# zkonduit/ezkl

Hardware: AMD Instinct MI355X
Metric: BN254 G1 MSM pts/s (2^20 points per GPU; NTT 2^22 elems/s in extra) (higher is better)
Workload: dtype u32x8 (254-bit modular integer, Montgomery); 1 GPU; configs[1]: standalone 2^20-point BN254 G1 MSM (uniform scalars, try-and-increment bases) + 2^22 scalar-field NTT per GPU; parallelism=points sharded across 1 rank(s); all_gather of 64-B partials + host fold

## Files before the change

### ezkl_amd/csrc/msm.hip

```cpp
#include "common.hpp"
#include <deque>
#include <thread>
#include <chrono>
#include "curve.hpp"
#include "curve29.hpp"
#include "host64.hpp"
#include <string.h>

namespace ezkl {

static constexpr uint32_t MSM_MAX_PART_BITS = 12;
static constexpr uint32_t MSM_SPAN_HEAVY = 16;
static constexpr uint32_t MSM_PART_STAGE = 13312;
static constexpr uint32_t MSM_BINSORT_STAGE = 15360;
static constexpr uint32_t MSM_HEAVY_CHUNK = 256;
static constexpr uint32_t MSM_DIGIT_E = 8;
static constexpr uint32_t MSM_LMIN = 8;
static constexpr uint32_t MSM_MAX_BIG = 64;
static constexpr uint32_t MSM_BIG_BLOCKS = 64;
static constexpr uint32_t MSM_BIG_ROWS = 8;

__device__ __forceinline__ uint32_t msm_part_of(uint32_t bucket, uint32_t NP) { return bucket ? 1u + (bucket & (NP - 1u)) : 0u; }
__device__ __forceinline__ uint32_t msm_lane_len(const uint32_t* offsets, uint32_t nb, uint32_t nlanes, uint32_t lmin) {
    const uint32_t l = (uint32_t)(((uint64_t)offsets[nb] + nlanes - 1) / nlanes);
// ... 155 lines not shown
        uint32_t raw = msm_take_bits(s, c) + carry;
        if (raw > half) {
            carry = 1;
            if (raw != (1u << c)) f(w, (1u << c) - raw - 1u, neg ^ 1u);
        } else {
            carry = 0;
            if (raw) f(w, raw - 1u, neg);
        }
    }
}

__device__ __forceinline__ bool msm_digit_step(fe_t& s, uint32_t neg, uint32_t c, uint32_t& carry, uint32_t& bucket, uint32_t& sign) {
    const uint32_t half = 1u << (c - 1);
    const uint32_t raw = msm_take_bits(s, c) + carry;
    if (raw > half) {
        carry = 1;
        bucket = (1u << c) - raw - 1u;
        sign = neg ^ 1u;
        return raw != (1u << c);
    }
    carry = 0;
    bucket = raw - 1u;
    sign = neg;
    return raw != 0;
}

__device__ __forceinline__ uint32_t msm_block_scan(uint32_t v, uint32_t* wsum, uint32_t& total) {
    const uint32_t lane = threadIdx.x & 63u, wave = threadIdx.x >> 6, nw = blockDim.x >> 6;
    uint32_t x = v;
#pragma unroll
    for (uint32_t d = 1; d < 64; d <<= 1) {
        const uint32_t y = __shfl_up(x, d, 64);
        if (lane >= d) x += y;
    }
    if (lane == 63) wsum[wave] = x;
    __syncthreads();
    if (wave == 0) {
        uint32_t s = lane < nw ? wsum[lane] : 0u;
#pragma unroll
        for (uint32_t d = 1; d < 16; d <<= 1) {
            const uint32_t y = __shfl_up(s, d, 64);
            if (lane >= d) s += y;
        }
        if (lane < nw) wsum[lane] = s;
    }
    __syncthreads();
    total = wsum[nw - 1];
    const uint32_t r = x + (wave ? wsum[wave - 1] : 0u);
    __syncthreads();
    return r;
}

__global__ __launch_bounds__(256) void msm_hist_kernel(const fe_t* scalars, size_t n, size_t per_block, WinPlan wp,
                                                       uint32_t LB, uint32_t NP, uint32_t* wg_hist, uint32_t* wg_cnt,
                                                       const fe_t* const* scal_list, uint32_t* zero_base, uint32_t zero_words, size_t bstride) {
    BOFF(); BSH(wg_hist); BSH(wg_cnt);
    if (scal_list) scalars = scal_list[blockIdx.z];
    if (zero_base) {
        BSH(zero_base);
        for (uint32_t i = blockIdx.x * 256 + threadIdx.x; i < zero_words; i += gridDim.x * 256) zero_base[i] = 0;
    }
    __shared__ uint32_t lh[(1u << MSM_MAX_PART_BITS) + 1];
    const uint32_t NQ = NP + 1;
    for (uint32_t p = threadIdx.x; p < NQ; p += 256) lh[p] = 0;
    __syncthreads();
    size_t lo = (size_t)blockIdx.x * per_block, hi = lo + per_block < n ? lo + per_block : n;
    for (size_t i0 = lo + threadIdx.x; i0 < hi; i0 += 4 * 256) {
        fe_t s[4];
        uint32_t neg[4], carry[4] = {0, 0, 0, 0};
#pragma unroll
        for (int q = 0; q < 4; q++) {
            const size_t i = i0 + (size_t)q * 256;
            if (i < hi) s[q] = msm_canon(scalars, i, neg[q]);
            else { s[q] = Fr::zero(); neg[q] = 0; }
        }
        for (uint32_t w = 0; w < wp.W; w++) {
            const uint32_t c = wp.width(w);
#pragma unroll
            for (int q = 0; q < 4; q++) {
                uint32_t bucket, sign;
                if (msm_digit_step(s[q], neg[q], c, carry[q], bucket, sign)) atomicAdd(&lh[msm_part_of(bucket, NP)], 1u);
            }
        }
    }
    __syncthreads();
    for (uint32_t p = threadIdx.x; p < NQ; p += 256) {
        wg_hist[(size_t)blockIdx.x * NQ + p] = lh[p];
        wg_cnt[(size_t)blockIdx.x * NQ + p] = lh[p];
    }
}
__global__ __launch_bounds__(1024) void msm_hist_scan_kernel(uint32_t* wg_hist, uint32_t G, uint32_t NP, uint32_t* part_count, size_t bstride) {
    BOFF(); BSH(wg_hist); BSH(part_count);
    __shared__ uint32_t sums[32][33];
    const uint32_t c = threadIdx.x & 31, j = threadIdx.x >> 5;
    const uint32_t p = blockIdx.x * 32 + c;
    const uint32_t chunk = (G + 31) / 32, g0 = j * chunk, g1 = g0 + chunk < G ? g0 + chunk : G;
    uint32_t s = 0;
    if (p < NP)
        for (uint32_t g = g0; g < g1; g++) s += wg_hist[(size_t)g * NP + p];
    sums[j][c] = s;
    __syncthreads();
    if (j == 0) {
        uint32_t run = 0;
        for (uint32_t q = 0; q < 32; q++) {
            uint32_t v = sums[q][c];
            sums[q][c] = run;
            run += v;
        }
        if (p < NP) part_count[p] = run;
    }
    __syncthreads();
    if (p < NP) {
        uint32_t run = sums[j][c];
        for (uint32_t g = g0; g < g1; g++) {
            uint32_t v = wg_hist[(size_t)g * NP + p];
            wg_hist[(size_t)g * NP + p] = run;
            run += v;
        }
    }
}
__device__ __forceinline__ void msm_part_scan_body(const uint32_t* part_count, uint32_t NQ, uint32_t* part_base, uint32_t* big_flag,
                                                   uint32_t* big_list, uint32_t* big_count, uint32_t* sh) {
    const uint32_t t = threadIdx.x;
    constexpr uint32_t PER = 5;
    uint32_t v[PER], sum = 0;
#pragma unroll
    for (uint32_t q = 0; q < PER; q++) {
        const uint32_t i = PER * t + q;
        v[q] = i < NQ ? part_count[i] : 0;
        sum += v[q];
    }
    uint32_t total;
    uint32_t run = msm_block_scan(sum, sh, total) - sum;
#pragma unroll
    for (uint32_t q = 0; q < PER; q++) {
        const uint32_t i = PER * t + q;
        if (i < NQ) part_base[i] = run;
        run += v[q];
    }
    if (t == 1023) part_base[NQ] = total;
#pragma unroll
    for (uint32_t q = 0; q < PER; q++) {
        const uint32_t i = PER * t + q;
        if (i == 0 || i >= NQ) continue;
        uint32_t slot = 0;
        if (v[q] > MSM_BINSORT_STAGE) {
            slot = atomicAdd(big_count, 1u);
            if (slot < MSM_MAX_BIG) big_list[slot] = i - 1;
            slot = slot < MSM_MAX_BIG ? slot + 1 : 0;
        }
        big_flag[i - 1] = slot;
    }
}
__global__ __launch_bounds__(1024) void msm_part_scan_kernel(const uint32_t* part_count, uint32_t NQ, uint32_t* part_base, uint32_t* big_flag,
                                                             uint32_t* big_list, uint32_t* big_count, size_t bstride) {
    BOFF(); BSH(part_count); BSH(part_base); BSH(big_flag); BSH(big_list); BSH(big_count);
    __shared__ uint32_t sh[1024];
    msm_part_scan_body(part_count, NQ, part_base, big_flag, big_list, big_count, sh);
}
__global__ __launch_bounds__(1024) void msm_partition_kernel(const fe_t* scalars, size_t n, size_t per_block, WinPlan wp,
                                                             uint32_t LB, uint32_t NP, size_t base_offset, size_t tab_stride,
                                                             const uint32_t* part_base, const uint32_t* wg_hist, const uint32_t* wg_cnt, uint2* entries,
                                                             uint32_t* vals, const fe_t* const* scal_list, size_t bstride) {
    BOFF(); BSH(part_base); BSH(wg_hist); BSH(wg_cnt); BSH(entries); BSH(vals);
    if (scal_list) scalars = scal_list[blockIdx.z];
    extern __shared__ uint32_t plds[];
    __shared__ uint32_t tsum[1024];
    const uint32_t NQ = NP + 1;
    uint32_t* start = plds;
    uint32_t* cursor = plds + (NQ + 1);
    uint32_t* gbase = plds + 2 * (NQ + 1);
    uint2* stage = reinterpret_cast<uint2*>(plds + 3 * (NQ + 1));
    const uint32_t t = threadIdx.x, T = blockDim.x;
    const uint32_t K = (NQ + T - 1) / T;
    uint32_t loc = 0;
    for (uint32_t q = 0; q < K; q++) {
        const uint32_t p = t * K + q;
        if (p < NQ) loc += wg_cnt[(size_t)blockIdx.x * NQ + p];
    }
    uint32_t total;
    uint32_t run = msm_block_scan(loc, tsum, total) - loc;
    for (uint32_t q = 0; q < K; q++) {
        const uint32_t p = t * K + q;
        if (p < NQ) {
            start[p] = run;
            cursor[p] = run;
            gbase[p] = part_base[p] + wg_hist[(size_t)blockIdx.x * NQ + p];
            run += wg_cnt[(size_t)blockIdx.x * NQ + p];
        }
    }
    __syncthreads();
    const size_t lo = (size_t)blockIdx.x * per_block, hi = lo + per_block < n ? lo + per_block : n;
    const size_t i = lo + t;
    if (i < hi) {
        uint32_t neg;
        fe_t s = msm_canon(scalars, i, neg);
        msm_foreach_digit(s, neg, wp, [&](uint32_t w, uint32_t bucket, uint32_t sign) {
            const uint32_t r = atomicAdd(&cursor[msm_part_of(bucket, NP)], 1u);
            stage[r] = make_uint2((uint32_t)(w * tab_stride + base_offset + i) | (sign << 31), bucket);
        });
    }
    __syncthreads();
    const uint32_t PB = 31 - __clz(NP);
    for (uint32_t idx = t; idx < total; idx += T) {
        const uint2 e = stage[idx];
        const uint32_t p = msm_part_of(e.y, NP);
        const uint32_t slot = gbase[p] + (idx - start[p]);
        if (p) entries[slot] = make_uint2(e.x, e.y >> PB);
        else vals[slot] = e.x;
    }
}
__device__ __forceinline__ uint32_t msm_wave_rank(uint32_t* cnt, uint32_t key) {
    const uint64_t active = __ballot(1);
    const uint32_t first = __builtin_amdgcn_readfirstlane(key);
    if (__ballot(key == first) == active) {
        const uint32_t rank = (uint32_t)__popcll(active & ((1ull << (threadIdx.x & 63u)) - 1ull));
        uint32_t base = 0;
        if (rank == 0) base = atomicAdd(&cnt[first], (uint32_t)__popcll(active));
        return (uint32_t)__builtin_amdgcn_readfirstlane(base) + rank;
    }
    return atomicAdd(&cnt[key], 1u);
}
__device__ __forceinline__ void msm_bins_scan(uint32_t* cnt, uint32_t* tsum, uint32_t nbins, uint32_t p, uint32_t beg, const uint32_t* part_base,
                                              bool emit, uint32_t* offsets, g1x29_t* buckets) {
    const uint32_t t = threadIdx.x;
    uint32_t loc[4], s = 0;
#pragma unroll
    for (int q = 0; q < 4; q++) {
        uint32_t j = t * 4 + q;
        loc[q] = j < nbins ? cnt[j] : 0;
        s += loc[q];
    }
    uint32_t total;
    uint32_t run = msm_block_scan(s, tsum, total) - s;
#pragma unroll
    for (int q = 0; q < 4; q++) {
        uint32_t j = t * 4 + q;
        if (j < nbins) {
            cnt[j] = run;
            if (emit) {
                const bool b0 = (p == 0 && j == 0);
                offsets[(size_t)p * nbins + j] = b0 ? part_base[0] : beg + run;
                if (b0 ? part_base[1] == part_base[0] : loc[q] == 0) st_f29(&buckets[(size_t)p * nbins + j].zz, Fq29::zero());
// ... 130 lines not shown
        uint32_t mid = (lo + hi) >> 1;
        if (offsets[mid] <= k0) lo = mid; else hi = mid;
    }
    uint32_t b = lo, bin_end = offsets[b + 1];
    uint32_t end_next = offsets[b + 2 <= nb ? b + 2 : nb];
    lane_first[t] = b;
    bool started_before = offsets[b] < k0;
    g1x29_t acc = g1x29_identity();
    MsmRec nxt = msm_fetch(tab, vals[k0]);
    uint32_t vn = k0 + 1 < k1 ? vals[k0 + 1] : 0u;
    for (uint32_t k = k0; k < k1; k++) {
        if (k == bin_end) {
            if (started_before) st_g1x29(head + t, acc); else st_g1x29(buckets + b, acc);
            acc.zz = Fq29::zero();
            started_before = false;
            b++;
            bin_end = end_next;
            if (bin_end == k) {
                uint32_t probes = 1;
                while (bin_end == k && probes < 4) { b++; bin_end = offsets[b + 1]; probes++; }
                if (bin_end == k) {
                    uint32_t lo2 = b + 1, hi2 = nb;
                    while (hi2 - lo2 > 1) {
                        uint32_t mid = (lo2 + hi2) >> 1;
                        if (offsets[mid] <= k) lo2 = mid; else hi2 = mid;
                    }
                    b = lo2;
                    bin_end = offsets[b + 1];
                }
            }
            end_next = offsets[b + 2 <= nb ? b + 2 : nb];
        }
        const MsmRec cur = nxt;
        nxt = msm_fetch(tab, vn);
        vn = k + 2 < k1 ? vals[k + 2] : 0u;
        acc = g1x29_add_mixed(acc, g1a29_unpack(cur.p), cur.neg);
    }
    if (k1 == bin_end) {
        if (started_before) st_g1x29(head + t, acc); else st_g1x29(buckets + b, acc);
    } else {
        if (started_before) st_g1x29(head + t, acc); else st_g1x29(tail + t, acc);
    }
}
EZ_D g1x29_t g1x29_shfl_down(const g1x29_t& p, uint32_t d) {
    g1x29_t r;
    const uint32_t* s = p.x.v;
    uint32_t* o = r.x.v;
#pragma unroll
    for (int k = 0; k < 36; k++) o[k] = __shfl_down(s[k], d);
    return r;
}
__global__ __launch_bounds__(256) void msm_fixup_boundary_tree_kernel(const uint32_t* offsets, uint32_t nb, uint32_t nlanes,
                                                                      const uint32_t* lane_first, const g1x29_t* head, const g1x29_t* tail, g1x29_t* buckets,
                                                                      uint32_t* heavy_list, uint32_t* heavy_count, uint32_t* chunk_list, uint32_t lmin,
                                                                      uint32_t span_heavy, size_t bstride) {
    BOFF(); BSH(offsets); BSH(lane_first); BSH(head); BSH(tail); BSH(buckets); BSH(heavy_list); BSH(heavy_count); BSH(chunk_list);
    const uint32_t t = blockIdx.x * blockDim.x + threadIdx.x + 1;
    const uint32_t lane = threadIdx.x & 63u;
    const uint32_t L = msm_lane_len(offsets, nb, nlanes, lmin);
    const uint64_t k0 = (uint64_t)t * L;
    bool cut = t < nlanes && k0 < offsets[nb];
    uint32_t b = 0, t1 = 0, t2 = 0;
    if (cut) {
        b = lane_first[t];
        const uint32_t beg = offsets[b], end = offsets[b + 1];
        cut = beg < k0;
        t1 = beg / L; t2 = (end - 1) / L;
    }
    if (cut && t2 - t1 > span_heavy) {
        if (t == t1 + 1 && t2 - t1 > MSM_HEAVY_CHUNK) heavy_list[atomicAdd(heavy_count, 1u)] = b;
        if ((t - t1 - 1) % MSM_HEAVY_CHUNK == 0) chunk_list[atomicAdd(heavy_count + 1, 1u)] = t;
        cut = false;
    }
    const uint32_t wave_last = t + (63u - lane);
    const uint32_t run = cut ? (t2 < wave_last ? t2 : wave_last) - t + 1u : 0u;
    uint32_t longest = run;
#pragma unroll
    for (uint32_t o = 32; o > 0; o >>= 1) {
        const uint32_t m = __shfl_xor(longest, o);
        longest = m > longest ? m : longest;
    }
    if (longest == 0) return;
    if (longest <= 2) {
        if (!cut || t != t1 + 1) return;
        g1x29_t acc = g1x29_add(ld_g1x29(tail + t1), ld_g1x29(head + t));
        for (uint32_t u = t + 1; u <= t2; u++) acc = g1x29_add(acc, ld_g1x29(head + u));
        st_g1x29(buckets + b, acc);
        return;
    }
    g1x29_t v = cut ? ld_g1x29(head + t) : g1x29_identity();
    uint32_t have = cut ? 1u : 0u;
#pragma unroll 1
    for (uint32_t d = 1; d < longest; d <<= 1) {
        const g1x29_t w = g1x29_shfl_down(v, d);
        const uint32_t hw = __shfl_down(have, d);
        if (have == d && run > d) {
            v = g1x29_add(v, w);
            have += hw;
        }
    }
    if (!cut || t != t1 + 1) return;
    g1x29_t acc = g1x29_add(ld_g1x29(tail + t1), v);
    for (uint32_t u = t + run; u <= t2; u++) acc = g1x29_add(acc, ld_g1x29(head + u));
    st_g1x29(buckets + b, acc);
}
__global__ __launch_bounds__(256) void msm_fixup_heavy1_kernel(const uint32_t* offsets, uint32_t nb, uint32_t nlanes, const uint32_t* lane_first, g1x29_t* head,
                                                               const g1x29_t* tail, g1x29_t* buckets, const uint32_t* chunk_list, const uint32_t* counts, uint32_t lmin,
                                                               uint32_t coop, size_t bstride) {
    BOFF(); BSH(offsets); BSH(lane_first); BSH(head); BSH(tail); BSH(buckets); BSH(chunk_list); BSH(counts);
    const uint32_t nchunks = counts[1], L = msm_lane_len(offsets, nb, nlanes, lmin);
    const uint32_t wave = threadIdx.x >> 6, lane = threadIdx.x & 63u;
    for (uint32_t ci = blockIdx.x * 4u + wave; ci < nchunks; ci += gridDim.x * 4u) {
        const uint32_t start = chunk_list[ci], b = lane_first[start];
        const uint32_t t2 = (offsets[b + 1] - 1) / L;
        const uint32_t stop = start + MSM_HEAVY_CHUNK - 1 < t2 ? start + MSM_HEAVY_CHUNK - 1 : t2;
        const uint32_t t1 = offsets[b] / L;
        const bool whole = t2 - t1 <= MSM_HEAVY_CHUNK;
        g1x29_t acc = (whole && lane == 63u) ? ld_g1x29(tail + t1) : g1x29_identity();
        for (uint32_t t = start + lane; t <= stop; t += 64) acc = g1x29_add(acc, ld_g1x29(head + t));
        acc = coop ? g1x29_group_sum_coop(acc, 64) : g1x29_group_sum(acc, 64);
        if (lane == 0) st_g1x29(whole ? buckets + b : head + start, acc);
    }
}
__global__ __launch_bounds__(256) void msm_fixup_heavy2_kernel(const uint32_t* offsets, uint32_t nb, uint32_t nlanes, const g1x29_t* head, const g1x29_t* tail,
                                                               const uint32_t* heavy_list, const uint32_t* counts, g1x29_t* buckets, uint32_t lmin, uint32_t coop, size_t bstride) {
    BOFF(); BSH(offsets); BSH(head); BSH(tail); BSH(heavy_list); BSH(counts); BSH(buckets);
    const uint32_t L = msm_lane_len(offsets, nb, nlanes, lmin);
    const uint32_t wave = threadIdx.x >> 6, lane = threadIdx.x & 63u;
    for (uint32_t h = blockIdx.x * 4u + wave; h < counts[0]; h += gridDim.x * 4u) {
        const uint32_t b = heavy_list[h];
        const uint32_t t1 = offsets[b] / L, t2 = (offsets[b + 1] - 1) / L;
        g1x29_t acc = lane == 63u ? ld_g1x29(tail + t1) : g1x29_identity();
        for (uint32_t t = t1 + 1 + lane * MSM_HEAVY_CHUNK; t <= t2; t += 64 * MSM_HEAVY_CHUNK) acc = g1x29_add(acc, ld_g1x29(head + t));
        acc = coop ? g1x29_group_sum_coop(acc, 64) : g1x29_group_sum(acc, 64);
        if (lane == 0) st_g1x29(buckets + b, acc);
    }
}

struct ReduceGeom {
    uint32_t wA, wB, wC;
    uint32_t wsA, wsB, wsC;
    uint32_t EA, GA, ET, GT;
};
__global__ __launch_bounds__(256, 2) void msm_reduce1_kernel(const g1x29_t* buckets, ReduceGeom g, g1x29_t* partA, g1x29_t* partT, size_t bstride) {
    BOFF(); BSH(buckets); BSH(partA); BSH(partT);
    const uint32_t idx = blockIdx.x * blockDim.x + threadIdx.x;
    g1x29_t acc = g1x29_identity();
    if (blockIdx.y == 0) {
        if (idx >= (g.GA << g.wA)) return;
        const uint32_t dA = idx & ((1u << g.wA) - 1u), grp = idx >> g.wA;
        for (uint32_t e = 0; e < g.EA; e++) acc = g1x29_add(acc, ld_g1x29(buckets + ((((size_t)grp * g.EA + e) << g.wA) | dA)));
        st_g1x29(partA + (size_t)dA * g.GA + grp, acc);
    } else {
        const uint32_t nT = 1u << (g.wB + g.wC);
        if (idx >= nT * g.GT) return;
        const uint32_t grp = idx % g.GT, t = idx / g.GT;
        for (uint32_t e = 0; e < g.ET; e++) acc = g1x29_add(acc, ld_g1x29(buckets + (((size_t)t << g.wA) | (e * g.GT + grp))));
        st_g1x29(partT + (size_t)t * g.GT + grp, acc);
    }
}
__global__ __launch_bounds__(64) void msm_reduce2_kernel(const g1x29_t* partA, const g1x29_t* partT, ReduceGeom g, g1x29_t* SA, g1x29_t* T, uint32_t lanesA,
                                                         uint32_t lanesT, uint32_t blocksA, uint32_t coop, size_t bstride) {
    BOFF(); BSH(partA); BSH(partT); BSH(SA); BSH(T);
    const bool isA = blockIdx.x < blocksA;
    const uint32_t lanes = isA ? lanesA : lanesT, per = 64 / lanes;
    const uint32_t o = (isA ? blockIdx.x : blockIdx.x - blocksA) * per + threadIdx.x / lanes, j = threadIdx.x % lanes;
    const uint32_t nout = isA ? (1u << g.wA) : (1u << (g.wB + g.wC)), G = isA ? g.GA : g.GT;
    g1x29_t acc = g1x29_identity();
    if (o < nout) {
        const g1x29_t* src = (isA ? partA : partT) + (size_t)o * G;
        for (uint32_t i = j; i < G; i += lanes) acc = g1x29_add(acc, ld_g1x29(src + i));
    }
    acc = (coop && lanes >= 4) ? g1x29_group_sum_coop(acc, lanes) : g1x29_group_sum(acc, lanes);
    if (j == 0 && o < nout) st_g1x29((isA ? SA : T) + o, acc);
}
__global__ __launch_bounds__(256) void msm_planes_kernel(const g1x29_t* SA, const g1x29_t* T, ReduceGeom g, g1x29_t* planes, g1x29_t* planes_host, uint32_t coop,
                                                         size_t bstride) {
    BOFF(); BSH(SA); BSH(T); BSH(planes);
    __shared__ uint4 sh[9 * 4];
    uint32_t id = blockIdx.x, field = 0, j = 0;
    if (id > 0) {
        id -= 1;
        if (id < g.wA) { field = 1; j = id; }
        else if (id < g.wA + g.wB) { field = 2; j = id - g.wA; }
        else { field = 3; j = id - g.wA - g.wB; }
// ... 150 lines not shown
    const size_t resident = (size_t)acc_blocks_per_cu * 256 * c->num_cus;
    const size_t load = npairs >> bits, per_lane = load * 9 / 10 > 40 ? load * 9 / 10 : 40;
    size_t rounds = npairs / (resident * per_lane);
    if (rounds < 1) rounds = 1;
    uint32_t L = (uint32_t)((npairs + resident * rounds - 1) / (resident * rounds));
    if (L < 8) L = 8;
    if (const char* e = getenv("EZKL_MSM_L")) {
        const int v = atoi(e);
        if (v > 0 && v < (1 << 20)) L = (uint32_t)v;
    }
    const uint32_t nlanes = cdiv(npairs, L);
    static const uint32_t lmin = [] { const char* e = getenv("EZKL_MSM_LMIN"); const int v = e ? atoi(e) : 0; return (uint32_t)(v >= 1 && v <= 4096 ? v : (int)MSM_LMIN); }();
    constexpr uint32_t coop = 7;
    static const uint32_t span_heavy = [] { const char* e = getenv("EZKL_MSM_SPAN"); const int v = e ? atoi(e) : 0; return (uint32_t)(v >= 1 && v <= 4096 ? v : (int)MSM_SPAN_HEAVY); }();
    ReduceGeom rg;
    memset(&rg, 0, sizeof rg);
    if (LB > 0) {
        rg.wA = LB; rg.wsA = PB;
        rg.wB = (PB + 1) / 2; rg.wsB = 0;
        rg.wC = PB - rg.wB; rg.wsC = rg.wB;
    } else {
        rg.wA = (bits + 2) / 3; rg.wsA = 0;
        rg.wB = (bits - rg.wA + 1) / 2; rg.wsB = rg.wA;
        rg.wC = bits - rg.wA - rg.wB; rg.wsC = rg.wA + rg.wB;
    }
    {
        const uint32_t rows = 1u << (rg.wB + rg.wC), cols = 1u << rg.wA;
        uint32_t E = MSM_DIGIT_E;
        if (const char* e = getenv("EZKL_MSM_E")) {
            const int v = atoi(e);
            if (v > 0 && v <= 1024 && (v & (v - 1)) == 0) E = (uint32_t)v;
        }
        rg.EA = rows < E ? rows : E; rg.GA = rows / rg.EA;
        rg.ET = cols < E ? cols : E; rg.GT = cols / rg.ET;
    }
    const uint32_t nA = 1u << rg.wA, nT = 1u << (rg.wB + rg.wC);
    const uint32_t n_partA = nA * rg.GA, n_partT = nT * rg.GT;
    const uint32_t nplanes = 1 + bits;
    size_t per_block = MSM_PART_STAGE / W / 64 * 64;
    {
        const size_t lds_words = (144u << 10) / 4, fixed = 3 * ((size_t)NP + 2);
        const size_t fit = lds_words > fixed ? (lds_words - fixed) / (2 * (size_t)W) / 64 * 64 : 64;
        if (per_block > fit) per_block = fit;
    }
    if (per_block > 1024) per_block = 1024;
    if (per_block < 64) per_block = 64;
    const unsigned sgrid = cdiv(n, per_block);
    auto al = [](size_t x) { return (x + 255) & ~(size_t)255; };
    size_t off = 0;
    auto carve = [&](size_t bytes) { size_t o = off; off += al(bytes); return o; };
    size_t o_list = carve(MSM_MAX_GROUP * sizeof(void*));
    size_t o_ent = carve(npairs * 8), o_vals = carve(npairs * 4), o_offs = carve(((size_t)nb + 1) * 4);
    const uint32_t NQ = NP + 1;
    size_t o_pcnt = carve((NQ + 1) * 4), o_pbase = carve((NQ + 1) * 4), o_wgh = carve((size_t)sgrid * NQ * 4), o_wgc = carve((size_t)sgrid * NQ * 4);
    size_t o_heavy = carve((size_t)nb * 4), o_chunks = carve(((size_t)nlanes + 1) * 4);
    const size_t nbins = (size_t)1 << LB;
    size_t o_hcnt = carve(256), o_btot = carve(MSM_MAX_BIG * nbins * 4), o_planes = carve((size_t)nplanes * sizeof(g1x29_t));
    const size_t zero_bytes = off - o_hcnt;
    size_t o_bflag = carve((size_t)NP * 4), o_blist = carve(MSM_MAX_BIG * 4),
           o_boff = carve((size_t)MSM_MAX_BIG * MSM_BIG_BLOCKS * nbins * 4);
    size_t o_lfirst = carve((size_t)nlanes * 4);
    size_t o_bkt = carve((size_t)nb * sizeof(g1x29_t));
    size_t o_head = carve((size_t)nlanes * sizeof(g1x29_t)), o_tail = carve((size_t)nlanes * sizeof(g1x29_t));
    size_t o_partA = carve((size_t)n_partA * sizeof(g1x29_t)), o_partT = carve((size_t)n_partT * sizeof(g1x29_t));
    size_t o_SA = carve((size_t)nA * sizeof(g1x29_t)), o_T = carve((size_t)nT * sizeof(g1x29_t));
    const size_t bstride = count > 1 ? off : 0;
    rc = slot_prepare(sl, off * count, count);
    if (rc) return rc;
    uint8_t* S = sl.scratch;
    const fe_t* const* scal_list = nullptr;
    if (count > 1) {
        for (size_t j = 0; j < count; j++) sl.list_pinned[j] = cols[j];
        EZ_HIP(hipMemcpyAsync(S + o_list, sl.list_pinned, count * sizeof(void*), hipMemcpyHostToDevice, st));
        scal_list = (const fe_t* const*)(S + o_list);
    }
    uint2* entries = (uint2*)(S + o_ent);
    uint32_t* vals = (uint32_t*)(S + o_vals);
    uint32_t* offs = (uint32_t*)(S + o_offs);
    uint32_t *pcnt = (uint32_t*)(S + o_pcnt), *pbase = (uint32_t*)(S + o_pbase), *wghist = (uint32_t*)(S + o_wgh), *wgcnt = (uint32_t*)(S + o_wgc);
    uint32_t *heavy = (uint32_t*)(S + o_heavy), *hcnt = (uint32_t*)(S + o_hcnt), *chunks = (uint32_t*)(S + o_chunks);
    uint32_t* lfirst = (uint32_t*)(S + o_lfirst);
    uint32_t *bflag = (uint32_t*)(S + o_bflag), *blist = (uint32_t*)(S + o_blist), *btot = (uint32_t*)(S + o_btot), *boff = (uint32_t*)(S + o_boff);
    uint32_t* bcnt = hcnt + 2;
    g1x29_t *bkt = (g1x29_t*)(S + o_bkt), *head = (g1x29_t*)(S + o_head), *tail = (g1x29_t*)(S + o_tail);
    g1x29_t *partA = (g1x29_t*)(S + o_partA), *partT = (g1x29_t*)(S + o_partT), *SA = (g1x29_t*)(S + o_SA), *TT = (g1x29_t*)(S + o_T);
    g1x29_t* planes = (g1x29_t*)(S + o_planes);

    hipEvent_t m0 = nullptr, m1 = nullptr, a0 = nullptr, a1 = nullptr;
    bool timed_chain = timed;
    if (timed) {
        const char* tm = getenv("EZKL_HIP_TIMING");
        if (tm && !strcmp(tm, "none")) timed = timed_chain = false;
        else if (tm && !strcmp(tm, "kernel")) timed_chain = false;
    }
    if (timed) {
        if (timed_chain && (rc = ev_pair(c, "msm", &m0, &m1))) return rc;
        if ((rc = ev_pair(c, "msm_accumulate", &a0, &a1))) return rc;
        if (timed_chain) EZ_HIP(hipEventRecord(m0, st));
    }
    hipLaunchKernelGGL(msm_hist_kernel, dim3(sgrid, 1, Z), dim3(256), 0, st, scalars, n, per_block, wp, LB, NP, wghist, wgcnt, scal_list, hcnt,
                       (uint32_t)(zero_bytes / 4), bstride);
    hipLaunchKernelGGL(msm_hist_scan_kernel, dim3(cdiv(NQ, 32), 1, Z), dim3(1024), 0, st, wghist, sgrid, NQ, pcnt, bstride);
    hipLaunchKernelGGL(msm_part_scan_kernel, dim3(1, 1, Z), dim3(1024), 0, st, pcnt, NQ, pbase, bflag, blist, bcnt, bstride);
    hipLaunchKernelGGL(msm_partition_kernel, dim3(sgrid, 1, Z), dim3((unsigned)per_block), (3 * ((size_t)NQ + 1) + 2 * per_block * W) * 4, st, scalars, n, per_block, wp,
                       LB, NP, base_offset, T->n, pbase, wghist, wgcnt, entries, vals, scal_list, bstride);
    hipLaunchKernelGGL(msm_binsort_kernel, dim3(NP + MSM_BIG_BLOCKS * MSM_BIG_ROWS, 1, Z), dim3(512), MSM_BINSORT_STAGE * 4, st, entries, pbase, LB, NP, bflag, offs,
                       vals, bkt, blist, bcnt, btot, boff, bstride);
    hipLaunchKernelGGL(msm_bigsort_scatter_kernel, dim3(MSM_BIG_BLOCKS, MSM_BIG_ROWS, Z), dim3(512), 0, st, entries, pbase, LB, blist, bcnt, btot, boff, offs,
                       vals, bkt, bstride);
    if (timed) EZ_HIP(hipEventRecord(a0, st));
    hipLaunchKernelGGL(msm_accumulate_kernel, dim3(cdiv(nlanes, 256), 1, Z), dim3(256), 0, st, T->tab, offs, vals, nb, nlanes, bkt, head, tail,
                       lfirst, lmin, bstride);
    if (timed) EZ_HIP(hipEventRecord(a1, st));
    if (nlanes > 1)
    {
        hipLaunchKernelGGL(msm_fixup_boundary_tree_kernel, dim3(cdiv(nlanes - 1, 256), 1, Z), dim3(256), 0, st, offs, nb, nlanes, lfirst, head, tail, bkt,
                           heavy, hcnt, chunks, lmin, span_heavy, bstride);
    }
    {
        size_t max_heavy = nlanes / span_heavy + 1;
        const size_t heavy_wgs = (max_heavy + 3) / 4;
        unsigned hb = (unsigned)(heavy_wgs < (size_t)c->num_cus * 4 ? heavy_wgs : (size_t)c->num_cus * 4);
        size_t max_chunks = nlanes / MSM_HEAVY_CHUNK + max_heavy;
        const size_t chunk_wgs = (max_chunks + 3) / 4;
        unsigned cb = (unsigned)(chunk_wgs < (size_t)c->num_cus * 4 ? chunk_wgs : (size_t)c->num_cus * 4);
        hipLaunchKernelGGL(msm_fixup_heavy1_kernel, dim3(cb, 1, Z), dim3(256), 0, st, offs, nb, nlanes, lfirst, head, tail, bkt, chunks, hcnt, lmin, coop & 4u, bstride);
        hipLaunchKernelGGL(msm_fixup_heavy2_kernel, dim3(hb, 1, Z), dim3(256), 0, st, offs, nb, nlanes, head, tail, heavy, hcnt, bkt, lmin, coop & 4u, bstride);
    }
    {
        const uint32_t th = n_partA > n_partT ? n_partA : n_partT;
        hipLaunchKernelGGL(msm_reduce1_kernel, dim3(cdiv(th, 256), 2, Z), dim3(256), 0, st, bkt, rg, partA, partT, bstride);
        auto pow2_le = [](uint32_t x) { uint32_t p = 1; while (p * 2 <= x) p *= 2; return p; };
        uint32_t lanesA = pow2_le(rg.GA < 64 ? rg.GA : 64), lanesT = pow2_le(rg.GT < 64 ? rg.GT : 64);
        auto waves = [&](uint32_t nout, uint32_t lanes) { return cdiv(nout, 64 / lanes); };
        while (waves(nA, lanesA) + waves(nT, lanesT) > (unsigned)c->num_cus * 4 && (lanesA > 1 || lanesT > 1)) {
            if (lanesT > 1 && waves(nT, lanesT) >= waves(nA, lanesA)) lanesT >>= 1; else if (lanesA > 1) lanesA >>= 1; else lanesT >>= 1;
        }
        const uint32_t blocksA = waves(nA, lanesA);
        hipLaunchKernelGGL(msm_reduce2_kernel, dim3(blocksA + waves(nT, lanesT), 1, Z), dim3(64), 0, st, partA, partT, rg, SA, TT, lanesA, lanesT, blocksA, coop & 1u, bstride);
        hipLaunchKernelGGL(msm_planes_kernel, dim3(nplanes, 1, Z), dim3(256), 0, st, SA, TT, rg, planes, (g1x29_t*)sl.pinned_dev,
                           coop & 10u, bstride);
    }
    EZ_HIP(hipGetLastError());
    if (getenv("EZKL_MSM_DEBUG")) {
        uint32_t hc = 0;
        EZ_HIP(hipMemcpyAsync(&hc, hcnt, 4, hipMemcpyDeviceToHost, st));
        EZ_HIP(hipStreamSynchronize(st));
        fprintf(stderr, "[msm] n=%zu W=%u bits=%u L=%u nlanes=%u heavy=%u\n", n, W, bits, L, nlanes, hc);
    }
    if (timed_chain) EZ_HIP(hipEventRecord(m1, st));
    EZ_HIP(hipEventRecord(sl.done, st));
    sl.bits = bits;
    sl.count = (uint32_t)count;
    sl.busy = true;
    return EZKL_OK;
}
static int msm_run_groups(Ctx* c, MsmTable* T, size_t base_offset, const fe_t* const* cols, size_t batch, size_t n, void* out_host,
                          const hipEvent_t* wait_ev, bool small_scalars) {
    const size_t G = msm_group_size(T, n, small_scalars, batch);
    static const bool dbg = getenv("EZKL_MSM_DEBUG") != nullptr;
    if (dbg) fprintf(stderr, "[ezkl_hip] msm batch: %zu columns of %zu points, %s scalars, groups of %zu\n", batch, n, small_scalars ? "witness-shaped" : "general", G);
    int rc = EZKL_OK;
    size_t gi = 0;
    for (size_t j0 = 0; j0 < batch && !rc; gi++) {
        size_t cnt = batch - j0 < G ? batch - j0 : G;
        if (wait_ev && j0 > 0) {
            const size_t left = batch - j0;
            cnt = left <= 2 ? 1 : std::min(G, (left + 1) / 2);
        }
        MsmSlot& sl = g_slots[gi % MSM_SLOTS];
        if (sl.busy) rc = msm_finish(sl);
        if (!rc) rc = slot_prepare(sl, 0);
        for (size_t j = 0; wait_ev && j < cnt && !rc; j++)
            if (hipStreamWaitEvent(sl.st, wait_ev[j0 + j], 0) != hipSuccess) rc = EZKL_ERR_HIP;
        if (!rc) {
            sl.out = (uint8_t*)out_host + 64 * j0;
            rc = msm_enqueue(c, sl, sl.st, T, base_offset, cols + j0, cnt, n, false);
        }
        j0 += cnt;
    }
    for (size_t k = 0; k < (size_t)MSM_SLOTS; k++) {
        MsmSlot& sl = g_slots[(gi + k) % MSM_SLOTS];
        if (!sl.busy) continue;
        if (!rc) rc = msm_finish(sl);
        else { (void)hipStreamSynchronize(sl.st); sl.busy = false; }
    }
    return rc;
}

struct MsmBatch;
static MsmBatch* g_open_batch_fwd();
int msm_run(Ctx* c, hipStream_t st, const Bases* b, size_t base_offset, const fe_t* scalars, size_t n, void* out_host) {
    if (g_open_batch_fwd()) return EZKL_ERR_INVALID;
    if (n == 0) { memset(out_host, 0, 64); return EZKL_OK; }
    MsmTable* T = nullptr;
    int rc = table_get(c, st, b, &T);
    if (rc) return rc;
    MsmSlot& sl = g_slots[0];
    if (sl.busy) return EZKL_ERR_INVALID;
    static const bool host_timing = getenv("EZKL_MSM_HOST_TIMING") != nullptr;
    if (!host_timing) {
// ... 451 lines not shown
```

Measured before the change: 802.4 million pts/s.

## Fuse MSM histogram scans into partition and merge heavy fixup kernels

Removes the duplicate per-block histogram write and replaces the column-scan kernel with a 2D-gridded scan over block rows, writing exclusive prefixes to a separate buffer. Folds the partition-base scan and big-partition flagging into the partition kernel, which each block recomputes redundantly and block 0 publishes. Merges the two heavy-bucket fixup kernels into one using a per-bucket completion counter, so the last chunk finisher does the final sum. This cuts kernel launches and serial steps but adds redundant scan work per partition block and atomics with threadfences.

```diff
diff --git a/ezkl_amd/csrc/msm.hip b/ezkl_amd/csrc/msm.hip
--- a/ezkl_amd/csrc/msm.hip
+++ b/ezkl_amd/csrc/msm.hip
@@ -231,9 +231,9 @@
 }
 
 __global__ __launch_bounds__(256) void msm_hist_kernel(const fe_t* scalars, size_t n, size_t per_block, WinPlan wp,
-                                                       uint32_t LB, uint32_t NP, uint32_t* wg_hist, uint32_t* wg_cnt,
+                                                       uint32_t LB, uint32_t NP, uint32_t* wg_cnt,
                                                        const fe_t* const* scal_list, uint32_t* zero_base, uint32_t zero_words, size_t bstride) {
-    BOFF(); BSH(wg_hist); BSH(wg_cnt);
+    BOFF(); BSH(wg_cnt);
     if (scal_list) scalars = scal_list[blockIdx.z];
     if (zero_base) {
         BSH(zero_base);
@@ -263,85 +263,58 @@
         }
     }
     __syncthreads();
-    for (uint32_t p = threadIdx.x; p < NQ; p += 256) {
-        wg_hist[(size_t)blockIdx.x * NQ + p] = lh[p];
-        wg_cnt[(size_t)blockIdx.x * NQ + p] = lh[p];
-    }
-}
-__global__ __launch_bounds__(1024) void msm_hist_scan_kernel(uint32_t* wg_hist, uint32_t G, uint32_t NP, uint32_t* part_count, size_t bstride) {
-    BOFF(); BSH(wg_hist); BSH(part_count);
-    __shared__ uint32_t sums[32][33];
-    const uint32_t c = threadIdx.x & 31, j = threadIdx.x >> 5;
-    const uint32_t p = blockIdx.x * 32 + c;
-    const uint32_t chunk = (G + 31) / 32, g0 = j * chunk, g1 = g0 + chunk < G ? g0 + chunk : G;
-    uint32_t s = 0;
-    if (p < NP)
-        for (uint32_t g = g0; g < g1; g++) s += wg_hist[(size_t)g * NP + p];
-    sums[j][c] = s;
+    for (uint32_t p = threadIdx.x; p < NQ; p += 256) wg_cnt[(size_t)blockIdx.x * NQ + p] = lh[p];
+}
+static constexpr uint32_t MSM_SCAN_COLS = 8, MSM_SCAN_RPT = 4, MSM_SCAN_ROWS = 1024 / MSM_SCAN_COLS * MSM_SCAN_RPT;
+__global__ __launch_bounds__(1024) void msm_hist_scan_kernel(const uint32_t* __restrict__ wg_cnt, uint32_t* __restrict__ wg_pre, uint32_t G, uint32_t NQ,
+                                                             uint32_t* part_count, size_t bstride) {
+    BOFF(); BSH(wg_cnt); BSH(wg_pre); BSH(part_count);
+    constexpr uint32_t J = 1024 / MSM_SCAN_COLS;
+    __shared__ uint32_t sums[MSM_SCAN_COLS][J + 1], above[MSM_SCAN_COLS][J + 1];
+    __shared__ uint32_t wtot[16], atot[16];
+    const uint32_t t = threadIdx.x, c = t % MSM_SCAN_COLS, j = t / MSM_SCAN_COLS;
+    const uint32_t p = blockIdx.x * MSM_SCAN_COLS + c;
+    const uint32_t gb = blockIdx.y * MSM_SCAN_ROWS, g0 = gb + j * MSM_SCAN_RPT;
+    uint32_t v[MSM_SCAN_RPT], s = 0, up = 0;
+#pragma unroll
+    for (uint32_t q = 0; q < MSM_SCAN_RPT; q++) {
+        v[q] = (p < NQ && g0 + q < G) ? wg_cnt[(size_t)(g0 + q) * NQ + p] : 0u;
+        s += v[q];
+    }
+    if (p < NQ)
+        for (uint32_t g = j; g < gb; g += J) up += wg_cnt[(size_t)g * NQ + p];
+    sums[c][j] = s;
+    above[c][j] = up;
     __syncthreads();
-    if (j == 0) {
-        uint32_t run = 0;
-        for (uint32_t q = 0; q < 32; q++) {
-            uint32_t v = sums[q][c];
-            sums[q][c] = run;
-            run += v;
-        }
-        if (p < NP) part_count[p] = run;
-    }
+    const uint32_t lane = t & 63u, wave = t >> 6, c2 = wave >> 1, j2 = t % J;
+    const uint32_t x = sums[c2][j2];
+    uint32_t incl = x, a = above[c2][j2];
+#pragma unroll
+    for (uint32_t d = 1; d < 64; d <<= 1) {
+        const uint32_t y = __shfl_up(incl, d, 64);
+        if (lane >= d) incl += y;
+        a += __shfl_xor(a, d, 64);
+    }
+    if (lane == 63) wtot[wave] = incl;
+    if (lane == 0) atot[wave] = a;
     __syncthreads();
-    if (p < NP) {
-        uint32_t run = sums[j][c];
-        for (uint32_t g = g0; g < g1; g++) {
-            uint32_t v = wg_hist[(size_t)g * NP + p];
-            wg_hist[(size_t)g * NP + p] = run;
-            run += v;
-        }
-    }
-}
-__device__ __forceinline__ void msm_part_scan_body(const uint32_t* part_count, uint32_t NQ, uint32_t* part_base, uint32_t* big_flag,
-                                                   uint32_t* big_list, uint32_t* big_count, uint32_t* sh) {
-    const uint32_t t = threadIdx.x;
-    constexpr uint32_t PER = 5;
-    uint32_t v[PER], sum = 0;
-#pragma unroll
-    for (uint32_t q = 0; q < PER; q++) {
-        const uint32_t i = PER * t + q;
-        v[q] = i < NQ ? part_count[i] : 0;
-        sum += v[q];
-    }
-    uint32_t total;
-    uint32_t run = msm_block_scan(sum, sh, total) - sum;
-#pragma unroll
-    for (uint32_t q = 0; q < PER; q++) {
-        const uint32_t i = PER * t + q;
-        if (i < NQ) part_base[i] = run;
+    const uint32_t base = atot[2 * c2] + atot[2 * c2 + 1] + ((wave & 1u) ? wtot[2 * c2] : 0u);
+    sums[c2][j2] = base + incl - x;
+    if (blockIdx.y == gridDim.y - 1 && j2 == J - 1 && blockIdx.x * MSM_SCAN_COLS + c2 < NQ) part_count[blockIdx.x * MSM_SCAN_COLS + c2] = base + incl;
+    __syncthreads();
+    uint32_t run = sums[c][j];
+#pragma unroll
+    for (uint32_t q = 0; q < MSM_SCAN_RPT; q++) {
+        if (p < NQ && g0 + q < G) wg_pre[(size_t)(g0 + q) * NQ + p] = run;
         run += v[q];
     }
-    if (t == 1023) part_base[NQ] = total;
-#pragma unroll
-    for (uint32_t q = 0; q < PER; q++) {
-        const uint32_t i = PER * t + q;
-        if (i == 0 || i >= NQ) continue;
-        uint32_t slot = 0;
-        if (v[q] > MSM_BINSORT_STAGE) {
-            slot = atomicAdd(big_count, 1u);
-            if (slot < MSM_MAX_BIG) big_list[slot] = i - 1;
-            slot = slot < MSM_MAX_BIG ? slot + 1 : 0;
-        }
-        big_flag[i - 1] = slot;
-    }
-}
-__global__ __launch_bounds__(1024) void msm_part_scan_kernel(const uint32_t* part_count, uint32_t NQ, uint32_t* part_base, uint32_t* big_flag,
-                                                             uint32_t* big_list, uint32_t* big_count, size_t bstride) {
-    BOFF(); BSH(part_count); BSH(part_base); BSH(big_flag); BSH(big_list); BSH(big_count);
-    __shared__ uint32_t sh[1024];
-    msm_part_scan_body(part_count, NQ, part_base, big_flag, big_list, big_count, sh);
 }
 __global__ __launch_bounds__(1024) void msm_partition_kernel(const fe_t* scalars, size_t n, size_t per_block, WinPlan wp,
                                                              uint32_t LB, uint32_t NP, size_t base_offset, size_t tab_stride,
-                                                             const uint32_t* part_base, const uint32_t* wg_hist, const uint32_t* wg_cnt, uint2* entries,
-                                                             uint32_t* vals, const fe_t* const* scal_list, size_t bstride) {
-    BOFF(); BSH(part_base); BSH(wg_hist); BSH(wg_cnt); BSH(entries); BSH(vals);
+                                                             const uint32_t* part_count, const uint32_t* wg_pre, const uint32_t* wg_cnt, uint2* entries,
+                                                             uint32_t* vals, const fe_t* const* scal_list, uint32_t* part_base, uint32_t* big_flag,
+                                                             uint32_t* big_list, uint32_t* big_count, size_t bstride) {
+    BOFF(); BSH(part_count); BSH(wg_pre); BSH(wg_cnt); BSH(entries); BSH(vals); BSH(part_base); BSH(big_flag); BSH(big_list); BSH(big_count);
     if (scal_list) scalars = scal_list[blockIdx.z];
     extern __shared__ uint32_t plds[];
     __shared__ uint32_t tsum[1024];
@@ -352,22 +325,42 @@
     uint2* stage = reinterpret_cast<uint2*>(plds + 3 * (NQ + 1));
     const uint32_t t = threadIdx.x, T = blockDim.x;
     const uint32_t K = (NQ + T - 1) / T;
-    uint32_t loc = 0;
-    for (uint32_t q = 0; q < K; q++) {
-        const uint32_t p = t * K + q;
-        if (p < NQ) loc += wg_cnt[(size_t)blockIdx.x * NQ + p];
-    }
-    uint32_t total;
-    uint32_t run = msm_block_scan(loc, tsum, total) - loc;
+    uint32_t loc = 0, ptot = 0;
     for (uint32_t q = 0; q < K; q++) {
         const uint32_t p = t * K + q;
         if (p < NQ) {
+            loc += wg_cnt[(size_t)blockIdx.x * NQ + p];
+            ptot += part_count[p];
+        }
+    }
+    uint32_t total, npairs;
+    uint32_t run = msm_block_scan(loc, tsum, total) - loc;
+    uint32_t pb = msm_block_scan(ptot, tsum, npairs) - ptot;
+    const bool first = blockIdx.x == 0;
+    for (uint32_t q = 0; q < K; q++) {
+        const uint32_t p = t * K + q;
+        if (p < NQ) {
+            const uint32_t pc = part_count[p];
             start[p] = run;
             cursor[p] = run;
-            gbase[p] = part_base[p] + wg_hist[(size_t)blockIdx.x * NQ + p];
+            gbase[p] = pb + wg_pre[(size_t)blockIdx.x * NQ + p];
             run += wg_cnt[(size_t)blockIdx.x * NQ + p];
-        }
-    }
+            if (first) {
+                part_base[p] = pb;
+                if (p) {
+                    uint32_t slot = 0;
+                    if (pc > MSM_BINSORT_STAGE) {
+                        slot = atomicAdd(big_count, 1u);
+                        if (slot < MSM_MAX_BIG) big_list[slot] = p - 1;
+                        slot = slot < MSM_MAX_BIG ? slot + 1 : 0;
+                    }
+                    big_flag[p - 1] = slot;
+                }
+            }
+            pb += pc;
+        }
+    }
+    if (first && t == 0) part_base[NQ] = npairs;
     __syncthreads();
     const size_t lo = (size_t)blockIdx.x * per_block, hi = lo + per_block < n ? lo + per_block : n;
     const size_t i = lo + t;
@@ -604,9 +597,9 @@
 }
 __global__ __launch_bounds__(256) void msm_fixup_boundary_tree_kernel(const uint32_t* offsets, uint32_t nb, uint32_t nlanes,
                                                                       const uint32_t* lane_first, const g1x29_t* head, const g1x29_t* tail, g1x29_t* buckets,
-                                                                      uint32_t* heavy_list, uint32_t* heavy_count, uint32_t* chunk_list, uint32_t lmin,
+                                                                      uint32_t* heavy_count, uint32_t* chunk_list, uint32_t lmin,
                                                                       uint32_t span_heavy, size_t bstride) {
-    BOFF(); BSH(offsets); BSH(lane_first); BSH(head); BSH(tail); BSH(buckets); BSH(heavy_list); BSH(heavy_count); BSH(chunk_list);
+    BOFF(); BSH(offsets); BSH(lane_first); BSH(head); BSH(tail); BSH(buckets); BSH(heavy_count); BSH(chunk_list);
     const uint32_t t = blockIdx.x * blockDim.x + threadIdx.x + 1;
     const uint32_t lane = threadIdx.x & 63u;
     const uint32_t L = msm_lane_len(offsets, nb, nlanes, lmin);
@@ -620,7 +613,6 @@
         t1 = beg / L; t2 = (end - 1) / L;
     }
     if (cut && t2 - t1 > span_heavy) {
-        if (t == t1 + 1 && t2 - t1 > MSM_HEAVY_CHUNK) heavy_list[atomicAdd(heavy_count, 1u)] = b;
         if ((t - t1 - 1) % MSM_HEAVY_CHUNK == 0) chunk_list[atomicAdd(heavy_count + 1, 1u)] = t;
         cut = false;
     }
@@ -656,10 +648,10 @@
     for (uint32_t u = t + run; u <= t2; u++) acc = g1x29_add(acc, ld_g1x29(head + u));
     st_g1x29(buckets + b, acc);
 }
-__global__ __launch_bounds__(256) void msm_fixup_heavy1_kernel(const uint32_t* offsets, uint32_t nb, uint32_t nlanes, const uint32_t* lane_first, g1x29_t* head,
-                                                               const g1x29_t* tail, g1x29_t* buckets, const uint32_t* chunk_list, const uint32_t* counts, uint32_t lmin,
-                                                               uint32_t coop, size_t bstride) {
-    BOFF(); BSH(offsets); BSH(lane_first); BSH(head); BSH(tail); BSH(buckets); BSH(chunk_list); BSH(counts);
+__global__ __launch_bounds__(256) void msm_fixup_heavy_kernel(const uint32_t* offsets, uint32_t nb, uint32_t nlanes, const uint32_t* lane_first, g1x29_t* head,
+                                                              const g1x29_t* tail, g1x29_t* buckets, const uint32_t* chunk_list, const uint32_t* counts, uint32_t* done,
+                                                              uint32_t lmin, uint32_t coop, size_t bstride) {
+    BOFF(); BSH(offsets); BSH(lane_first); BSH(head); BSH(tail); BSH(buckets); BSH(chunk_list); BSH(counts); BSH(done);
     const uint32_t nchunks = counts[1], L = msm_lane_len(offsets, nb, nlanes, lmin);
     const uint32_t wave = threadIdx.x >> 6, lane = threadIdx.x & 63u;
     for (uint32_t ci = blockIdx.x * 4u + wave; ci < nchunks; ci += gridDim.x * 4u) {
@@ -672,17 +664,15 @@
         for (uint32_t t = start + lane; t <= stop; t += 64) acc = g1x29_add(acc, ld_g1x29(head + t));
         acc = coop ? g1x29_group_sum_coop(acc, 64) : g1x29_group_sum(acc, 64);
         if (lane == 0) st_g1x29(whole ? buckets + b : head + start, acc);
-    }
-}
-__global__ __launch_bounds__(256) void msm_fixup_heavy2_kernel(const uint32_t* offsets, uint32_t nb, uint32_t nlanes, const g1x29_t* head, const g1x29_t* tail,
-                                                               const uint32_t* heavy_list, const uint32_t* counts, g1x29_t* buckets, uint32_t lmin, uint32_t coop, size_t bstride) {
-    BOFF(); BSH(offsets); BSH(head); BSH(tail); BSH(heavy_list); BSH(counts); BSH(buckets);
-    const uint32_t L = msm_lane_len(offsets, nb, nlanes, lmin);
-    const uint32_t wave = threadIdx.x >> 6, lane = threadIdx.x & 63u;
-    for (uint32_t h = blockIdx.x * 4u + wave; h < counts[0]; h += gridDim.x * 4u) {
-        const uint32_t b = heavy_list[h];
-        const uint32_t t1 = offsets[b] / L, t2 = (offsets[b + 1] - 1) / L;
-        g1x29_t acc = lane == 63u ? ld_g1x29(tail + t1) : g1x29_identity();
+        if (whole) continue;
+        uint32_t last = 0;
+        if (lane == 0) {
+            __threadfence();
+            last = atomicAdd(&done[t1 / MSM_HEAVY_CHUNK], 1u) + 1u == (t2 - t1 + MSM_HEAVY_CHUNK - 1) / MSM_HEAVY_CHUNK ? 1u : 0u;
+        }
+        if (!__shfl(last, 0, 64)) continue;
+        __threadfence();
+        acc = lane == 63u ? ld_g1x29(tail + t1) : g1x29_identity();
         for (uint32_t t = t1 + 1 + lane * MSM_HEAVY_CHUNK; t <= t2; t += 64 * MSM_HEAVY_CHUNK) acc = g1x29_add(acc, ld_g1x29(head + t));
         acc = coop ? g1x29_group_sum_coop(acc, 64) : g1x29_group_sum(acc, 64);
         if (lane == 0) st_g1x29(buckets + b, acc);
@@ -939,10 +929,11 @@
     size_t o_list = carve(MSM_MAX_GROUP * sizeof(void*));
     size_t o_ent = carve(npairs * 8), o_vals = carve(npairs * 4), o_offs = carve(((size_t)nb + 1) * 4);
     const uint32_t NQ = NP + 1;
-    size_t o_pcnt = carve((NQ + 1) * 4), o_pbase = carve((NQ + 1) * 4), o_wgh = carve((size_t)sgrid * NQ * 4), o_wgc = carve((size_t)sgrid * NQ * 4);
-    size_t o_heavy = carve((size_t)nb * 4), o_chunks = carve(((size_t)nlanes + 1) * 4);
+    size_t o_pcnt = carve((NQ + 1) * 4), o_pbase = carve((NQ + 1) * 4), o_wgp = carve((size_t)sgrid * NQ * 4), o_wgc = carve((size_t)sgrid * NQ * 4);
+    size_t o_chunks = carve(((size_t)nlanes + 1) * 4);
     const size_t nbins = (size_t)1 << LB;
-    size_t o_hcnt = carve(256), o_btot = carve(MSM_MAX_BIG * nbins * 4), o_planes = carve((size_t)nplanes * sizeof(g1x29_t));
+    size_t o_hcnt = carve(256), o_hdone = carve(((size_t)nlanes / MSM_HEAVY_CHUNK + 1) * 4), o_btot = carve(MSM_MAX_BIG * nbins * 4),
+           o_planes = carve((size_t)nplanes * sizeof(g1x29_t));
     const size_t zero_bytes = off - o_hcnt;
     size_t o_bflag = carve((size_t)NP * 4), o_blist = carve(MSM_MAX_BIG * 4),
            o_boff = carve((size_t)MSM_MAX_BIG * MSM_BIG_BLOCKS * nbins * 4);
@@ -964,8 +955,8 @@
     uint2* entries = (uint2*)(S + o_ent);
     uint32_t* vals = (uint32_t*)(S + o_vals);
     uint32_t* offs = (uint32_t*)(S + o_offs);
-    uint32_t *pcnt = (uint32_t*)(S + o_pcnt), *pbase = (uint32_t*)(S + o_pbase), *wghist = (uint32_t*)(S + o_wgh), *wgcnt = (uint32_t*)(S + o_wgc);
-    uint32_t *heavy = (uint32_t*)(S + o_heavy), *hcnt = (uint32_t*)(S + o_hcnt), *chunks = (uint32_t*)(S + o_chunks);
+    uint32_t *pcnt = (uint32_t*)(S + o_pcnt), *pbase = (uint32_t*)(S + o_pbase), *wgpre = (uint32_t*)(S + o_wgp), *wgcnt = (uint32_t*)(S + o_wgc);
+    uint32_t *hcnt = (uint32_t*)(S + o_hcnt), *hdone = (uint32_t*)(S + o_hdone), *chunks = (uint32_t*)(S + o_chunks);
     uint32_t* lfirst = (uint32_t*)(S + o_lfirst);
     uint32_t *bflag = (uint32_t*)(S + o_bflag), *blist = (uint32_t*)(S + o_blist), *btot = (uint32_t*)(S + o_btot), *boff = (uint32_t*)(S + o_boff);
     uint32_t* bcnt = hcnt + 2;
@@ -985,12 +976,11 @@
         if ((rc = ev_pair(c, "msm_accumulate", &a0, &a1))) return rc;
         if (timed_chain) EZ_HIP(hipEventRecord(m0, st));
     }
-    hipLaunchKernelGGL(msm_hist_kernel, dim3(sgrid, 1, Z), dim3(256), 0, st, scalars, n, per_block, wp, LB, NP, wghist, wgcnt, scal_list, hcnt,
+    hipLaunchKernelGGL(msm_hist_kernel, dim3(sgrid, 1, Z), dim3(256), 0, st, scalars, n, per_block, wp, LB, NP, wgcnt, scal_list, hcnt,
                        (uint32_t)(zero_bytes / 4), bstride);
-    hipLaunchKernelGGL(msm_hist_scan_kernel, dim3(cdiv(NQ, 32), 1, Z), dim3(1024), 0, st, wghist, sgrid, NQ, pcnt, bstride);
-    hipLaunchKernelGGL(msm_part_scan_kernel, dim3(1, 1, Z), dim3(1024), 0, st, pcnt, NQ, pbase, bflag, blist, bcnt, bstride);
+    hipLaunchKernelGGL(msm_hist_scan_kernel, dim3(cdiv(NQ, MSM_SCAN_COLS), cdiv(sgrid, MSM_SCAN_ROWS), Z), dim3(1024), 0, st, wgcnt, wgpre, sgrid, NQ, pcnt, bstride);
     hipLaunchKernelGGL(msm_partition_kernel, dim3(sgrid, 1, Z), dim3((unsigned)per_block), (3 * ((size_t)NQ + 1) + 2 * per_block * W) * 4, st, scalars, n, per_block, wp,
-                       LB, NP, base_offset, T->n, pbase, wghist, wgcnt, entries, vals, scal_list, bstride);
+                       LB, NP, base_offset, T->n, pcnt, wgpre, wgcnt, entries, vals, scal_list, pbase, bflag, blist, bcnt, bstride);
     hipLaunchKernelGGL(msm_binsort_kernel, dim3(NP + MSM_BIG_BLOCKS * MSM_BIG_ROWS, 1, Z), dim3(512), MSM_BINSORT_STAGE * 4, st, entries, pbase, LB, NP, bflag, offs,
                        vals, bkt, blist, bcnt, btot, boff, bstride);
     hipLaunchKernelGGL(msm_bigsort_scatter_kernel, dim3(MSM_BIG_BLOCKS, MSM_BIG_ROWS, Z), dim3(512), 0, st, entries, pbase, LB, blist, bcnt, btot, boff, offs,
@@ -1002,17 +992,14 @@
     if (nlanes > 1)
     {
         hipLaunchKernelGGL(msm_fixup_boundary_tree_kernel, dim3(cdiv(nlanes - 1, 256), 1, Z), dim3(256), 0, st, offs, nb, nlanes, lfirst, head, tail, bkt,
-                           heavy, hcnt, chunks, lmin, span_heavy, bstride);
+                           hcnt, chunks, lmin, span_heavy, bstride);
     }
     {
-        size_t max_heavy = nlanes / span_heavy + 1;
-        const size_t heavy_wgs = (max_heavy + 3) / 4;
-        unsigned hb = (unsigned)(heavy_wgs < (size_t)c->num_cus * 4 ? heavy_wgs : (size_t)c->num_cus * 4);
-        size_t max_chunks = nlanes / MSM_HEAVY_CHUNK + max_heavy;
+        const size_t max_chunks = nlanes / MSM_HEAVY_CHUNK + nlanes / span_heavy + 1;
         const size_t chunk_wgs = (max_chunks + 3) / 4;
         unsigned cb = (unsigned)(chunk_wgs < (size_t)c->num_cus * 4 ? chunk_wgs : (size_t)c->num_cus * 4);
-        hipLaunchKernelGGL(msm_fixup_heavy1_kernel, dim3(cb, 1, Z), dim3(256), 0, st, offs, nb, nlanes, lfirst, head, tail, bkt, chunks, hcnt, lmin, coop & 4u, bstride);
-        hipLaunchKernelGGL(msm_fixup_heavy2_kernel, dim3(hb, 1, Z), dim3(256), 0, st, offs, nb, nlanes, head, tail, heavy, hcnt, bkt, lmin, coop & 4u, bstride);
+        hipLaunchKernelGGL(msm_fixup_heavy_kernel, dim3(cb, 1, Z), dim3(256), 0, st, offs, nb, nlanes, lfirst, head, tail, bkt, chunks, hcnt, hdone, lmin, coop & 4u,
+                           bstride);
     }
     {
         const uint32_t th = n_partA > n_partT ? n_partA : n_partT;
@@ -1031,9 +1018,9 @@
     EZ_HIP(hipGetLastError());
     if (getenv("EZKL_MSM_DEBUG")) {
         uint32_t hc = 0;
-        EZ_HIP(hipMemcpyAsync(&hc, hcnt, 4, hipMemcpyDeviceToHost, st));
+        EZ_HIP(hipMemcpyAsync(&hc, hcnt + 1, 4, hipMemcpyDeviceToHost, st));
         EZ_HIP(hipStreamSynchronize(st));
-        fprintf(stderr, "[msm] n=%zu W=%u bits=%u L=%u nlanes=%u heavy=%u\n", n, W, bits, L, nlanes, hc);
+        fprintf(stderr, "[msm] n=%zu W=%u bits=%u L=%u nlanes=%u heavy_chunks=%u\n", n, W, bits, L, nlanes, hc);
     }
     if (timed_chain) EZ_HIP(hipEventRecord(m1, st));
     EZ_HIP(hipEventRecord(sl.done, st));
```

After: 808.6 million pts/s (median of 6 runs). No clear change (+0.8%).
